# ericzzj1989/BALF

Measured on NVIDIA B200. Metric: images/sec detect+NMS+top-k @640x480, higher is better.
Workload: dtype fp16/tf32 operands (11-bit significand), fp32 accumulate

## Files before the change

### balf_b200/csrc/detector_tc.cuh

```cuda
#pragma once
#include <cuda_fp16.h>
#include "detector.cuh"
#include "umma.cuh"

namespace balf {
using namespace umma;

constexpr int kMerge32Ctas = 3;
constexpr int kRc16MinC = 32;
constexpr int TM = 128;
constexpr int NT2 = 256;
constexpr int kMaxSlot = 4;
constexpr int kMaxGemm = 6;

struct TcGemm {
    uint32_t goff;
    uint16_t nblk;
    uint16_t rows;
    uint16_t kb;
    uint16_t bias;
    uint16_t h16;
};
__host__ __device__ constexpr uint32_t tc_eb(int h16) { return h16 == 1 ? 2u : 4u; }
struct TcPlan {
    const float* base;
    TcGemm g[kMaxGemm];
    int ngemm;
    int resident;
    uint32_t bytes;
    uint32_t slot_bytes;
    uint32_t nslot;
    uint32_t ebias_off;
    long long* trace;
};
#ifdef BALF_TC_MAIN
long long* g_tc_trace = nullptr;
int g_tc_trace_sel = 0;
#else
extern long long* g_tc_trace;
extern int g_tc_trace_sel;
#endif
constexpr int kTracePoints = 16, kTraceTiles = 16;
#ifdef BALF_TC_TRACE
#define TC_TRACE(plan, it, pt)                                                                                     \
    do {                                                                                                           \
        if ((plan).trace && blockIdx.x == 0 && (it) < kTraceTiles && (threadIdx.x == 0 || threadIdx.x == NT2 - 1)) \
            (plan).trace[(((it) * kTracePoints + (pt)) << 1) + (threadIdx.x ? 1 : 0)] = clock64();                 \
    } while (0)
#else
#define TC_TRACE(plan, it, pt) do { (void)(it); } while (0)
#endif

enum { BG_CONV0 = 0, BG_PD1, BG_D1A, BG_D1B, BG_WM, BG_D2, BG_COUNT };
enum { MG_CONV0 = 0, MG_PD2A, MG_PD2B, MG_RC1, MG_RC2, MG_COUNT };
enum { HG_C2 = 0, HG_DENSE, HG_COUNT };
constexpr int kHeadN = 80;

__host__ __device__ constexpr int tc_kin(int cin) { return cin < 8 ? 8 : cin; }
__host__ __device__ constexpr int tc_kb(int rows, int K, int cap = 32768, int eb = 4) {
    int kb = K;
    while (kb > 32 / eb && (kb * rows * eb > cap || K % kb != 0)) kb /= 2;
    return kb;
}
__host__ __device__ constexpr int tc_cols(int need) { return need <= 32 ? 32 : need <= 64 ? 64 : need <= 128 ? 128 : need <= 256 ? 256 : 512; }
__host__ __device__ inline uint32_t gemm_block_bytes(const TcGemm& g, uint32_t b) {
    return (uint32_t)g.rows * (g.kb * tc_eb(g.h16) + ((g.bias && b + 1 == g.nblk) ? 32u : 0u));
}
__host__ __device__ inline uint32_t gemm_bytes(const TcGemm& g) {
    return (uint32_t)g.rows * ((uint32_t)g.kb * g.nblk * tc_eb(g.h16) + (g.bias ? 32u : 0u));
}

struct Ring {
    uint32_t wsm;
    uint64_t* full;
    uint64_t* empty;
    uint32_t pidx, nsched;
    const uint2* sched;
    uint32_t pcnt, ccnt;
    uint32_t pslot, puse;
    uint32_t cslot, cpar;
    uint32_t to_load;
};

__device__ __forceinline__ void bulk_load(uint32_t dst, const float* src, uint32_t bytes, uint64_t* bar) {
    asm volatile("cp.async.bulk.shared::cluster.global.mbarrier::complete_tx::bytes [%0], [%1], %2, [%3];"
                 :: "r"(dst), "l"(src), "r"(bytes), "r"(smem_u32(bar)) : "memory");
}
__device__ __forceinline__ void ring_build_schedule(uint2* sched, const TcPlan& p, uint32_t* count) {
    uint32_t n = 0;
    for (int gi = 0; gi < p.ngemm; ++gi) {
        const TcGemm g = p.g[gi];
        for (uint32_t b = 0; b < g.nblk; ++b)
            sched[n++] = make_uint2(g.goff + b * (uint32_t)g.rows * g.kb / (g.h16 == 1 ? 2u : 1u), gemm_block_bytes(g, b));
    }
    *count = n;
}
template <int NS>
__device__ __forceinline__ void ring_load_one(Ring& r, const TcPlan& p) {
    const uint2 e = r.sched[r.pidx];
    const uint32_t slot = r.pslot;
    if (r.puse > 0) mbar_wait(&r.empty[slot], (r.puse - 1) & 1);
    mbar_expect_tx(&r.full[slot], e.y);
    bulk_load(r.wsm + slot * p.slot_bytes, p.base + e.x, e.y, &r.full[slot]);
    ++r.pcnt;
    --r.to_load;
    if (++r.pslot == NS) { r.pslot = 0; ++r.puse; }
    if (++r.pidx == r.nsched) r.pidx = 0;
}
template <int NS>
__device__ __forceinline__ void ring_top_up(Ring& r, const TcPlan& p) {
    while (r.to_load > 0 && r.pcnt < r.ccnt + NS) ring_load_one<NS>(r, p);
}
template <int NS>
__device__ __forceinline__ void ring_consumed(Ring& r) {
    ++r.ccnt;
    if (++r.cslot == NS) { r.cslot = 0; r.cpar ^= 1; }
}
__device__ __forceinline__ void ring_load_all(Ring& r, const TcPlan& p) {
    mbar_expect_tx(&r.full[0], p.bytes);
    uint32_t off = 0;
    for (int gi = 0; gi < p.ngemm; ++gi) {
        const uint32_t bytes = gemm_bytes(p.g[gi]);
        bulk_load(r.wsm + off, p.base + p.g[gi].goff, bytes, &r.full[0]);
        off += bytes;
    }
}
template <int CIN, int C, int PX = 0> struct BranchG {
    static constexpr int count = BG_COUNT;
    static constexpr bool x3 = PX != 0;
    static constexpr bool resident = PX ? C <= 64 : C <= 128;
    static constexpr int cap = 32768;
    static constexpr int nslot = PX ? (C == 256 ? 2 : 3) : (C == 256 ? 3 : 2);
    __host__ __device__ static constexpr int rows(int gi) { return gi == BG_WM ? 64 : C; }
    __host__ __device__ static constexpr int K(int gi) { return gi == BG_CONV0 ? tc_kin(CIN) : gi == BG_WM ? 64 : C; }
    __host__ __device__ static constexpr bool bias(int gi) { return gi != BG_WM; }
    __host__ __device__ static constexpr bool h16(int gi) { return gi != BG_CONV0 || CIN >= 8; }
};
template <int CIN, int C, int PX = 0> struct MergeG {
    static constexpr int count = MG_COUNT;
    static constexpr bool x3 = PX != 0;
    static constexpr bool ebias = C == 128 && PX == 0;
    static constexpr bool resident = PX ? C <= 32 : C <= 128;
    static constexpr int cap = 32768;
    static constexpr int nslot = PX ? (C == 64 ? 3 : 2) : (C == 256 ? 2 : 3);
    __host__ __device__ static constexpr int rows(int) { return C; }
    __host__ __device__ static constexpr int K(int gi) { return gi == MG_CONV0 ? tc_kin(CIN) : C; }
    __host__ __device__ static constexpr bool bias(int gi) { return !ebias && gi != MG_PD2A; }
    __host__ __device__ static constexpr bool h16(int gi) {
        return gi == MG_PD2A || gi == MG_PD2B || (gi == MG_CONV0 && CIN >= 8) || ((gi == MG_RC1 || gi == MG_RC2) && (PX || C > kRc16MinC));
    }
};
template <int C, int PX = 0> struct HeadG {
    static constexpr int count = HG_COUNT;
    static constexpr bool x3 = PX != 0;
    static constexpr bool resident = false;
    static constexpr int cap = 32768;
    static constexpr int nslot = 2;
    __host__ __device__ static constexpr int rows(int gi) { return gi == HG_DENSE ? kHeadN : C; }
    __host__ __device__ static constexpr int K(int) { return C; }
    __host__ __device__ static constexpr bool bias(int) { return true; }
    __host__ __device__ static constexpr bool h16(int) { return true; }
};
template <typename G> __host__ __device__ constexpr int g_mode(int gi) { return G::h16(gi) ? (G::x3 ? 2 : 1) : 0; }
template <typename G> __host__ __device__ constexpr uint32_t g_bytes(int gi) {
    return (uint32_t)G::rows(gi) * (G::K(gi) * tc_eb(g_mode<G>(gi)) + (G::bias(gi) ? 32u : 0u));
}
template <typename G> __host__ __device__ constexpr uint32_t g_off(int gi) { uint32_t o = 0; for (int i = 0; i < gi; ++i) o += g_bytes<G>(i); return o; }

constexpr uint32_t kDescHi = (128u >> 4) | (1u << 14);
__device__ __forceinline__ uint64_t desc_of(uint32_t addr, uint32_t lbo) {
    return ((uint64_t)kDescHi << 32) | (uint64_t)(((lbo >> 4) << 16) | ((addr >> 4) & 0x3FFFu));
}

__host__ __device__ constexpr uint32_t make_idesc_f16(int M, int N) { return (1u << 4) | ((uint32_t)(N >> 3) << 17) | ((uint32_t)(M >> 4) << 24); }
__device__ __forceinline__ void mma_f16(uint32_t d_tmem, uint64_t a_desc, uint64_t b_desc, uint32_t idesc, bool accumulate) {
    asm volatile(
        "{\n\t.reg .pred p;\n\tsetp.ne.b32 p, %4, 0;\n\t"
        "tcgen05.mma.cta_group::1.kind::f16 [%0], %1, %2, %3, p;\n\t}"
        :: "r"(d_tmem), "l"(a_desc), "l"(b_desc), "r"(idesc), "r"((uint32_t)accumulate) : "memory");
}
constexpr uint32_t kDescHiSw = (1024u >> 4) | (1u << 14) | (2u << 29);
__device__ __forceinline__ uint64_t desc_sw_of(uint32_t addr) {
    return ((uint64_t)kDescHiSw << 32) | (uint64_t)((1u << 16) | ((addr >> 4) & 0x3FFFu));
}
template <typename G, int GI, bool ASW = false>
__device__ __forceinline__ void issue_linear_t(Ring& r, const TcPlan& p, uint32_t a_addr, uint32_t ones_addr, uint32_t d_tmem, bool first) {
    constexpr int ROWS = G::rows(GI), K = G::K(GI);
    constexpr bool BIAS = G::bias(GI), H16 = G::h16(GI);
    constexpr bool X3 = H16 && G::x3;
    static_assert(!(H16 && ASW), "fp16 operands use the chunk-major layout");
    constexpr int KB = tc_kb(ROWS, K, G::cap, (int)tc_eb(g_mode<G>(GI))), NBLK = K / KB;
    constexpr uint32_t idesc = H16 ? make_idesc_f16(128, ROWS) : make_idesc_tf32(128, ROWS);
    constexpr uint32_t a_lbo = TM * 16u, b_lbo = (uint32_t)ROWS * 16u;
    constexpr int KSTEP = H16 ? 16 : 8, EPC = H16 ? 8 : 4;
    const uint64_t a_desc = ASW ? desc_sw_of(a_addr) : desc_of(a_addr, a_lbo);
#pragma unroll
    for (int b = 0; b < NBLK; ++b) {
        uint32_t w_addr, slot = 0;
        if (G::resident) {
            w_addr = r.wsm + g_off<G>(GI) + (uint32_t)b * ROWS * KB * tc_eb(g_mode<G>(GI));
        } else {
            ring_top_up<G::nslot>(r, p);
            slot = r.cslot;
            mbar_wait(&r.full[slot], r.cpar);
            w_addr = r.wsm + slot * p.slot_bytes;
        }
        const uint64_t b_desc = desc_of(w_addr, b_lbo);
        fence_after_sync();
#pragma unroll
        for (int ks = 0; ks < KB / KSTEP; ++ks) {
            const uint32_t kchunk = (uint32_t)(b * KB) / EPC + (uint32_t)ks * 2u;
            const uint32_t a_off = ASW ? (kchunk / 8u) * (TM * 128u) + (kchunk % 8u) * 16u : kchunk * a_lbo;
            if (H16) mma_f16(d_tmem, a_desc + (a_off >> 4), b_desc + (((uint32_t)ks * 2u * b_lbo) >> 4), idesc, !(first && b == 0 && ks == 0));
            else mma_tf32(d_tmem, a_desc + (a_off >> 4), b_desc + (((uint32_t)ks * 2u * b_lbo) >> 4), idesc, !(first && b == 0 && ks == 0));
            if constexpr (X3) {
                mma_f16(d_tmem, a_desc + ((a_off + (uint32_t)(K / 8) * a_lbo) >> 4), b_desc + (((uint32_t)ks * 2u * b_lbo) >> 4), idesc, true);
                mma_f16(d_tmem, a_desc + (a_off >> 4), b_desc + ((((uint32_t)KB / 8u + (uint32_t)ks * 2u) * b_lbo) >> 4), idesc, true);
            }
        }
        if (BIAS && b + 1 == NBLK)
            mma_tf32(d_tmem, desc_of(ones_addr, TM * 16u), b_desc + ((((uint32_t)KB / EPC) * (X3 ? 2u : 1u) * b_lbo) >> 4), make_idesc_tf32(128, ROWS), true);
        if (!G::resident) { commit(&r.empty[slot]); ring_consumed<G::nslot>(r); }
    }
}

constexpr uint32_t kDescHiMn = ((uint32_t)(TM * 16u) >> 4) | (1u << 14);
__device__ __forceinline__ uint64_t desc_mn_of(uint32_t addr) {
    return ((uint64_t)kDescHiMn << 32) | (uint64_t)(((128u >> 4) << 16) | ((addr >> 4) & 0x3FFFu));
}
template <typename G, int GI, int C>
__device__ __forceinline__ void issue_mix_t(Ring& r, const TcPlan& p, uint32_t y_addr, uint32_t d_tmem) {
    uint32_t w_addr, slot = 0;
    if (G::resident) {
        w_addr = r.wsm + g_off<G>(GI);
    } else {
        ring_top_up<G::nslot>(r, p);
        slot = r.cslot;
        mbar_wait(&r.full[slot], r.cpar);
        w_addr = r.wsm + slot * p.slot_bytes;
    }
    fence_after_sync();
    constexpr uint32_t idesc = make_idesc_f16(64, C) | (1u << 16);
    constexpr uint32_t lo_off = (uint32_t)(C / 8) * TM * 16u;
    const uint64_t w_desc = desc_of(w_addr, 1024u);
    const uint64_t y_desc = desc_mn_of(y_addr);
#pragma unroll
    for (uint32_t u = 0; u < 2; ++u) {
#pragma unroll
        for (uint32_t ks = 0; ks < 4; ++ks) {
            const uint32_t yo = (32u * ks + 16u * u) * 16u;
            mma_f16(d_tmem + ((u * 16u) << 16), w_desc + ((ks * 2u * 1024u) >> 4), y_desc + (yo >> 4), idesc, ks > 0);
            if constexpr (G::x3) {
                mma_f16(d_tmem + ((u * 16u) << 16), w_desc + ((ks * 2u * 1024u) >> 4), y_desc + ((lo_off + yo) >> 4), idesc, true);
                mma_f16(d_tmem + ((u * 16u) << 16), w_desc + ((8192u + ks * 2u * 1024u) >> 4), y_desc + (yo >> 4), idesc, true);
            }
        }
    }
    if (!G::resident) { commit(&r.empty[slot]); ring_consumed<G::nslot>(r); }
}

__device__ __forceinline__ float ex2_approx(float x) {
    float y;
    asm("ex2.approx.ftz.f32 %0, %1;" : "=f"(y) : "f"(x));
    return y;
}
__device__ __forceinline__ unsigned long long pk2(float lo, float hi) {
    unsigned long long r;
    asm("mov.b64 %0, {%1, %2};" : "=l"(r) : "f"(lo), "f"(hi));
    return r;
}
__device__ __forceinline__ void upk2(unsigned long long r, float& lo, float& hi) { asm("mov.b64 {%0, %1}, %2;" : "=f"(lo), "=f"(hi) : "l"(r)); }
__device__ __forceinline__ unsigned long long fma2(unsigned long long a, unsigned long long b, unsigned long long c) {
    unsigned long long d;
    asm("fma.rn.f32x2 %0, %1, %2, %3;" : "=l"(d) : "l"(a), "l"(b), "l"(c));
    return d;
}
__device__ __forceinline__ unsigned long long add2(unsigned long long a, unsigned long long b) {
    unsigned long long d;
    asm("add.rn.f32x2 %0, %1, %2;" : "=l"(d) : "l"(a), "l"(b));
    return d;
}
__device__ __forceinline__ unsigned long long mul2(unsigned long long a, unsigned long long b) {
    unsigned long long d;
    asm("mul.rn.f32x2 %0, %1, %2;" : "=l"(d) : "l"(a), "l"(b));
    return d;
}
__device__ __forceinline__ void gelu_erf2(float& v0, float& v1) {
    const float t0 = fmaxf(-fabsf(v0), -5.6568542494923806f), t1 = fmaxf(-fabsf(v1), -5.6568542494923806f);
    const unsigned long long t = pk2(t0, t1);
    unsigned long long p = fma2(pk2(3.586947569e-04f, 3.586947569e-04f), t, pk2(6.316647399e-03f, 6.316647399e-03f));
    p = fma2(p, t, pk2(5.013782158e-02f, 5.013782158e-02f));
// ... 157 lines not shown
    uint64_t* bars = reinterpret_cast<uint64_t*>(q);
    s.full = bars;
    s.empty = bars + kMaxSlot;
    s.done = bars + 2 * kMaxSlot;
    s.aux = bars + 2 * kMaxSlot + 1;
    s.tmem_slot = reinterpret_cast<uint32_t*>(bars + 2 * kMaxSlot + 2);
    s.gdone = bars + 2 * kMaxSlot + 3;
    return s;
}

template <int NS>
__device__ __forceinline__ void tc_prologue(const TcShared& s, uint32_t ncols, Ring& ring, const TcPlan& plan, uint32_t my_tiles, bool w0) {
    if (threadIdx.x < 32) tmem_alloc(s.tmem_slot, ncols);
    if (threadIdx.x == 0) {
        for (int i = 0; i < kMaxSlot; ++i) { mbar_init(&s.full[i], 1); mbar_init(&s.empty[i], 1); }
        mbar_init(s.done, 1);
        mbar_init(s.aux, 1);
        for (int i = 0; i < kMaxGroups; ++i) mbar_init(&s.gdone[i], 1);
        mbar_fence_init();
    }
    for (int i = threadIdx.x; i < 2 * TM; i += blockDim.x)
        reinterpret_cast<float4*>(s.ones)[i] = i < TM ? make_float4(1.f, 1.f, 0.f, 0.f) : make_float4(0.f, 0.f, 0.f, 0.f);
    fence_async_smem();
    fence_before_sync();
    __syncthreads();
    fence_after_sync();
    ring.wsm = s.wsm; ring.full = s.full; ring.empty = s.empty; ring.sched = s.sched;
    ring.pidx = ring.pcnt = ring.ccnt = 0;
    ring.pslot = ring.puse = ring.cslot = ring.cpar = 0;
    uint32_t nb = 0;
    for (int i = 0; i < plan.ngemm; ++i) nb += plan.g[i].nblk;
    ring.nsched = nb;
    ring.to_load = nb * my_tiles;
    if (w0 && elect_one()) {
        if (plan.resident) { ring_load_all(ring, plan); mbar_wait(&s.full[0], 0); }
        else {
            uint32_t cnt;
            ring_build_schedule(s.sched, plan, &cnt);
            ring_top_up<NS>(ring, plan);
        }
    }
}
__device__ __forceinline__ void tc_finish(uint32_t tm, uint32_t ncols) {
    fence_before_sync();
    __syncthreads();
    if (threadIdx.x < 32) tmem_dealloc(tm, ncols);
}
template <int NG = 1, int NTG = NT2>
__device__ __forceinline__ void sync_for_mma(int grp = 0) {
    fence_async_smem();
    fence_before_sync();
    group_sync<NG, NTG>(grp);
    fence_after_sync();
}
__device__ __forceinline__ void wait_done(uint64_t* done, uint32_t& phase) {
    if (threadIdx.x == 0) mbar_wait(done, phase & 1);
    __syncthreads();
    ++phase;
    fence_after_sync();
}
template <typename G, int NG = 1, int NTG = NT2>
__device__ __forceinline__ void wait_done_ring(uint64_t* done, uint32_t& phase, Ring& r, const TcPlan& p, bool w0, int grp = 0) {
    if (w0 && elect_one()) {
        mbar_wait(done, phase & 1);
        if (!G::resident) ring_top_up<G::nslot>(r, p);
    }
// ... 326 lines not shown
    const uint32_t lane_base = tm + ((uint32_t)(row & ~31) << 16);
    const uint32_t region_addr = smem_u32(s.region), ones_addr = smem_u32(s.ones);
    const int ug = (row & 31) >> 4, tok = (row >> 5) * 16 + (row & 15);
    const int col0 = half * CH;
    const float* const mix_b1p = s.vec + 512 + tok;
    const int ostride = (BR == 0 ? geo.fw : 1) * C;
    const size_t npix = (size_t)geo.h * geo.w;
    uint32_t phase = 0, xb = 0;
    int it = 0;
    InputPf<CIN, TPR> pf;
    auto coords = [&](int tt, bool& vld, int& im, int& px) {
        const int un = 2 * tt + ug;
        vld = un < geo.total_units;
        im = vld ? fast_div(un, geo.upi, geo.inv_upi) : 0;
        px = unit_pixel<BR>(geo, vld ? un - im * geo.upi : 0, tok);
    };
    auto stats_of = [&](const float (&v)[CH], float& sum, float& sq) {
        unsigned long long s2 = pk2(0.f, 0.f), q2 = pk2(0.f, 0.f);
#pragma unroll
        for (int i = 0; i < CH; i += 2) {
            const unsigned long long x = pk2(v[i], v[i + 1]);
            s2 = add2(s2, x); q2 = fma2(x, x, q2);
        }
        float a, b;
        upk2(s2, a, b); sum = a + b;
        upk2(q2, a, b); sq = a + b;
    };
    bool nvld = false; int nim = 0, npx = 0;
    if (InputPf<CIN, TPR>::enabled && vblock < ntiles) {
        coords(vblock, nvld, nim, npx);
        fetch_input_row<CIN, true, TPR, XH>(xin, npix, (size_t)nim, npx, nvld, half, pf);
    }
    for (int t = vblock; t < ntiles; t += vgrid, ++it) {
        TC_TRACE(plan, it, 0);
        bool valid; int img, pix;
        if (InputPf<CIN, TPR>::enabled && (TPR > 1 || !X3)) { valid = nvld; img = nim; pix = npx; }
        else coords(t, valid, img, pix);
        float* orow = rt + ((size_t)img * npix + pix) * C + col0;
        float v[CH], rstd, shift;
        if constexpr (CIN < 8) {
            const float4 xv = pf.v[0];
            if (t + vgrid < ntiles) {
                coords(t + vgrid, nvld, nim, npx);
                fetch_input_row<CIN, true, TPR, XH>(xin, npix, (size_t)nim, npx, nvld, half, pf);
            }
            conv0_row<CIN, C, CH>(xv, s.vec, col0, v);
        } else {
            if (InputPf<CIN, TPR>::enabled) {
                store_input_row<CIN, true, TPR, XM>(pf, s.region, row, half);
                if (t + vgrid < ntiles) {
                    coords(t + vgrid, nvld, nim, npx);
                    fetch_input_row<CIN, true, TPR, XH>(xin, npix, (size_t)nim, npx, nvld, half, pf);
                }
            } else {
                load_input_row<CIN, TPR, XM>(xin, npix, (size_t)img, pix, valid, s.region, row, half);
            }
            TC_TRACE(plan, it, 1);
            sync_for_mma<NG, NTG>(grp);
            if (w0 && elect_one()) { issue_linear_t<G, BG_CONV0>(ring, plan, region_addr, ones_addr, tm + Cfg::col_y, true); commit(s.done); }
            TC_TRACE(plan, it, 2);
            wait_done_ring<G, NG, NTG>(s.done, phase, ring, plan, w0, grp);
            TC_TRACE(plan, it, 3);
            ld_row<CH>(lane_base + Cfg::col_y + col0, v);
#pragma unroll
            for (int i = 0; i < CH; ++i) v[i] = fmaxf(v[i], 0.f);
        }
// ... 140 lines not shown
                        float4 t8[8];
                        pair_load<8>(reinterpret_cast<const float4*>(orow + c) + j0, valid, t8);
#pragma unroll
                        for (int j = 0; j < 8; j += 2) { pair_unswap(t8[j], t8[j + 1]); rq[j0 + j] = t8[j]; rq[j0 + j + 1] = t8[j + 1]; }
                    }
                }
#pragma unroll
                for (int j = 0; j < SC / 4; ++j) {
                    float4 res;
                    res = make_float4(r[4 * j], r[4 * j + 1], r[4 * j + 2], r[4 * j + 3]);
                    o[j] = make_float4(a[4 * j] + res.x, a[4 * j + 1] + res.y, a[4 * j + 2] + res.z, a[4 * j + 3] + res.w);
                    if (BR == 1 && !X3) o[j] = to_tf32_clean(o[j]);
                }
                if constexpr (SC % 32 == 0 && !X3) {
                    oct_store<SC / 4>(out, ((size_t)img * npix + pix) * C + col0 + c, ostride, reinterpret_cast<const float*>(o), valid);
                    continue;
                }
#pragma unroll
                for (int j = 0; j < SC / 4; j += 2) {
                    const float4 send = odd ? o[j] : o[j + 1];
                    float4 recv;
                    recv.x = __shfl_xor_sync(0xffffffffu, send.x, 1); recv.y = __shfl_xor_sync(0xffffffffu, send.y, 1);
                    recv.z = __shfl_xor_sync(0xffffffffu, send.z, 1); recv.w = __shfl_xor_sync(0xffffffffu, send.w, 1);
                    const float4 to_a = odd ? recv : o[j], to_b = odd ? o[j + 1] : recv;
                    const int chunk = (col0 + c) / 4 + j + (odd ? 1 : 0);
                    if (valid) {
                        *reinterpret_cast<float4*>(out + base_a + 4 * chunk) = to_a;
                        *reinterpret_cast<float4*>(out + base_b + 4 * chunk) = to_b;
                    }
                }
            }
        }
    }
    tc_finish(*s.tmem_slot, tc_cols(Cfg::ncols * NG));
}

template <int CIN, int C, int BR, int PX>
__global__ void __launch_bounds__(BranchCfg<C, PX>::NTG * BranchCfg<C, PX>::groups, 1)
tc_branch_kernel(const float* __restrict__ xin, DownW w, TcPlan plan, UnitGeom geo, float* __restrict__ out, float* __restrict__ scratch) {
    extern __shared__ __align__(1024) unsigned char smem[];
    tc_branch_body<CIN, C, BR, PX>(xin, w, plan, geo, out, scratch, smem);
}


template <int C, int NTH = NT2>
__device__ __forceinline__ void unit_channel_sums(const float* reg, int t, int total_units, float* __restrict__ partial) {
    constexpr int CQ = C / 4, PAIRS = 2 * CQ, TPP = NTH / PAIRS, RPT = 64 / TPP;
    static_assert(TPP >= 2 && TPP <= 16, "group must fit in a warp");
    const int tid = threadIdx.x, pair = tid / TPP, sub = tid % TPP;
    const int uu = pair / CQ, ch = pair % CQ;
    const float4* src = reinterpret_cast<const float4*>(reg) + (size_t)ch * TM + uu * 64 + sub;
    float4 acc = src[0];
#pragma unroll
    for (int i = 1; i < RPT; ++i) {
        const float4 x = src[i * TPP];
        acc.x += x.x; acc.y += x.y; acc.z += x.z; acc.w += x.w;
    }
#pragma unroll
    for (int o = TPP / 2; o >= 1; o >>= 1) {
        acc.x += __shfl_xor_sync(0xffffffffu, acc.x, o);
        acc.y += __shfl_xor_sync(0xffffffffu, acc.y, o);
        acc.z += __shfl_xor_sync(0xffffffffu, acc.z, o);
        acc.w += __shfl_xor_sync(0xffffffffu, acc.w, o);
    }
    const int un = 2 * t + uu;
    if (sub == 0 && un < total_units) *reinterpret_cast<float4*>(partial + (size_t)un * C + ch * 4) = acc;
// ... 42 lines not shown
    }
    const float* const eb = s.vec + col0_of(tid, CH);
    const uint32_t lane_base = tm + ((uint32_t)(row & ~31) << 16);
    const uint32_t region_addr = smem_u32(s.region), ones_addr = smem_u32(s.ones);
    const uint32_t r2_addr = region_addr + Cfg::r2_off;
    uint64_t* const ld_u = s.aux;
    uint64_t* const ld_v = &s.gdone[1];
    constexpr uint32_t kTileBytes = Cfg::uv_bytes;
    const size_t tile_floats = (size_t)kTileBytes / 4;
    uint32_t ld_phase = 0;
    const int ug = row >> 6, tok = row & 63;
    const int col0 = half * CH;
    const size_t npix = (size_t)geo.h * geo.w;
    uint32_t phase = 0, xb = 0;
    int it = 0;
    InputPf<CIN, TPR> pf;
    InputPf<C> pfu;
    auto coords = [&](int tt, bool& vld, int& im, int& px) {
        const int un = 2 * tt + ug;
        vld = un < geo.total_units;
        im = vld ? fast_div(un, geo.upi, geo.inv_upi) : 0;
        px = (vld ? un - im * geo.upi : 0) * 64 + tok;
    };
    if (InputPf<CIN, TPR>::enabled && (int)blockIdx.x < ntiles) {
        bool vld; int im, px;
        coords(blockIdx.x, vld, im, px);
        fetch_input_row<CIN, true, TPR, XH>(xin, npix, (size_t)im, px, vld, half, pf);
    }
    if (Cfg::bulk_uv && (int)blockIdx.x < ntiles && w0 && elect_one()) {
        mbar_expect_tx(ld_u, kTileBytes);
        bulk_load(r2_addr, uin + (size_t)blockIdx.x * tile_floats, kTileBytes, ld_u);
    }
    for (int t = blockIdx.x; t < ntiles; t += gridDim.x, ++it) {
        TC_TRACE(plan, it, 0);
        bool valid; int img, pix;
        coords(t, valid, img, pix);
        const size_t row_off = ((size_t)img * npix + pix) * C + col0;
        float v[CH];
        if (InputPf<CIN, TPR>::enabled) {
            store_input_row<CIN, true, TPR, XM>(pf, s.region, row, half);
            if (t + (int)gridDim.x < ntiles) {
                bool vld; int im, px;
                coords(t + gridDim.x, vld, im, px);
                fetch_input_row<CIN, true, TPR, XH>(xin, npix, (size_t)im, px, vld, half, pf);
            }
        } else {
            load_input_row<CIN, TPR, XM>(xin, npix, (size_t)img, pix, valid, s.region, row, half, PX ? 0 : CIN);
        }
        if (InputPf<C>::enabled) fetch_input_row<C>(uin, npix, (size_t)img, pix, valid, half, pfu);
        TC_TRACE(plan, it, 1);
        sync_for_mma();
        if constexpr (Cfg::bulk_uv) {
            if (w0 && elect_one()) {
                issue_linear_t<G, MG_CONV0>(ring, plan, region_addr, ones_addr, tm + Cfg::col_x0, true);
                mbar_wait(ld_u, ld_phase & 1);
                fence_after_sync();
                issue_linear_t<G, MG_PD2A>(ring, plan, r2_addr, ones_addr, tm + Cfg::col_acc, true);
                commit(s.done);
            }
            wait_done_ring<G>(s.done, phase, ring, plan, w0);
            if (w0 && elect_one()) {
                mbar_expect_tx(ld_v, kTileBytes);
                bulk_load(region_addr, vin + (size_t)t * tile_floats, kTileBytes, ld_v);
                if (!Cfg::two && t + (int)gridDim.x < ntiles) {
                    mbar_expect_tx(ld_u, kTileBytes);
                    bulk_load(r2_addr, uin + (size_t)(t + gridDim.x) * tile_floats, kTileBytes, ld_u);
// ... 99 lines not shown
            const float4 o = make_float4(v[4 * j], v[4 * j + 1], v[4 * j + 2], v[4 * j + 3]);
            *reinterpret_cast<float4*>(s.region + ((size_t)(col0 / 4 + j) * TM + row) * 4) = o;
        }
        static_assert(PX != 0 || C < 128 || CH % 64 == 0, "the fp16 r store (r16, decided by the host) assumes two threads per row");
        if constexpr (CH % 64 == 0 && PX == 0) {
            if (r16) {
                float hv[CH / 2];
#pragma unroll
                for (int i = 0; i < CH / 2; ++i) {
                    uint32_t h;
                    asm("cvt.rn.satfinite.f16x2.f32 %0, %1, %2;" : "=r"(h) : "f"(v[2 * i + 1]), "f"(v[2 * i]));
                    hv[i] = __uint_as_float(h);
                }
                oct_store<CH / 8>(rout, row_off / 2, C / 2, hv, valid);
            } else {
                oct_store<CH / 4>(rout, row_off, C, v, valid);
            }
        } else if constexpr (CH % 32 == 0 && PX == 0) {
            oct_store<CH / 4>(rout, row_off, C, v, valid);
        } else {
            pair_store<CH / 4>(rout, row_off, v, valid);
        }
        __syncthreads();
        unit_channel_sums<C, NTK>(s.region, t, geo.total_units, partial);
        if constexpr (Cfg::two) fence_async_smem();
        __syncthreads();
        if constexpr (Cfg::two) {
            if (t + (int)gridDim.x < ntiles && w0 && elect_one()) {
                mbar_expect_tx(ld_u, kTileBytes);
                bulk_load(r2_addr, uin + (size_t)(t + gridDim.x) * tile_floats, kTileBytes, ld_u);
            }
        }
    }
    tc_finish(tm, Cfg::ncols);
}


template <int CIN, int C, int PX = 0> struct MergeBulkCfg {
    static constexpr int CH = C / 2;
    static constexpr bool cc0 = CIN < 8;
    static constexpr uint32_t tile_bytes = (uint32_t)TM * C * 4;
    static constexpr uint32_t uv_bytes = (uint32_t)TM * C * (PX ? 4u : 2u);
    static constexpr uint32_t r16_bytes = 0u;
    static constexpr uint32_t xbytes = cc0 ? 0u : (uint32_t)TM * tc_kin(CIN) * 4;
    static constexpr uint32_t region = 2 * uv_bytes + r16_bytes + 2 * tile_bytes + xbytes;
    static constexpr uint32_t xch = 2u * TM * 8u;
    static constexpr int col_acc = 0, col_x0 = C;
    static constexpr int ncols = tc_cols(cc0 ? C : 2 * C);
    static constexpr int min_ctas = C <= 32 ? (PX ? 2 : kMerge32Ctas) : 1;
};

template <int CIN, int C, int PX = 0>
__global__ void __launch_bounds__(NT2, MergeBulkCfg<CIN, C, PX>::min_ctas)
tc_merge_bulk_kernel(const float* __restrict__ xin, DownW w, TcPlan plan, UnitGeom geo, const float* __restrict__ uin,
                     const float* __restrict__ vin, float* __restrict__ rout, float* __restrict__ qout, float* __restrict__ partial) {
    extern __shared__ __align__(1024) unsigned char smem[];
    using Cfg = MergeBulkCfg<CIN, C, PX>;
    constexpr int CH = Cfg::CH;
    using G = MergeG<CIN, C, PX>;
    constexpr int HM = PX ? 2 : 1, LOC = PX ? C / 8 : 0;
    constexpr bool XH = PX == 0 && CIN >= 8;
    constexpr int XM = XH ? 3 : HM;
    const TcShared s = carve(smem, Cfg::region, plan, 1, Cfg::xch);
    float* const regU = s.region;
    float* const regV = regU + Cfg::uv_bytes / 4;
    float* const regW = regV + Cfg::uv_bytes / 4;
// ... 152 lines not shown
            bulk_commit();
        }
        {
            constexpr int CQ = C / 4, TPP = NT2 / (2 * CQ), RPT = 64 / TPP;
            const int pair = tid / TPP, sub = tid % TPP;
            const int uu = pair / CQ, ch = pair % CQ;
            float4 acc = *reinterpret_cast<const float4*>(regW + sw_off(uu * 64 + sub, ch));
#pragma unroll
            for (int i = 1; i < RPT; ++i) {
                const float4 x = *reinterpret_cast<const float4*>(regW + sw_off(uu * 64 + sub + i * TPP, ch));
                acc.x += x.x; acc.y += x.y; acc.z += x.z; acc.w += x.w;
            }
#pragma unroll
            for (int o = TPP / 2; o >= 1; o >>= 1) {
                acc.x += __shfl_xor_sync(0xffffffffu, acc.x, o);
                acc.y += __shfl_xor_sync(0xffffffffu, acc.y, o);
                acc.z += __shfl_xor_sync(0xffffffffu, acc.z, o);
                acc.w += __shfl_xor_sync(0xffffffffu, acc.w, o);
            }
            if (sub == 0) *reinterpret_cast<float4*>(partial + (size_t)(2 * t + uu) * C + ch * 4) = acc;
        }
    }
    if (w0 && elect_one()) bulk_wait_all();
    tc_finish(tm, Cfg::ncols);
}

template <int C, int PX = 0>
__global__ void __launch_bounds__(NT2, 1) tc_head_kernel(const float* __restrict__ r, const float* __restrict__ q,
                                                         const float* __restrict__ scale, TcPlan plan, UnitGeom geo, int cell,
                                                         float* __restrict__ logits, float* __restrict__ prob, int r16) {
    extern __shared__ __align__(1024) unsigned char smem[];
    using G = HeadG<C, PX>;
    constexpr int LOC = PX ? C / 8 : 0;
    constexpr uint32_t region_bytes = (uint32_t)TM * C * 4;
    constexpr int ncols = tc_cols(C + 96);
    constexpr int CH = C / 2;
    const TcShared s = carve(smem, region_bytes, plan);
    const int tid = threadIdx.x, row = tid & (TM - 1), half = tid >> 7;
    const int ntiles = (geo.total_units + 1) / 2;
    const uint32_t my_tiles = blockIdx.x < (unsigned)ntiles ? (ntiles - 1 - blockIdx.x) / gridDim.x + 1 : 0;
    Ring ring;
    const bool w0 = warp0_uniform();
    tc_prologue<G::nslot>(s, ncols, ring, plan, my_tiles, w0);
    const uint32_t tm = *s.tmem_slot;
    const uint32_t lane_base = tm + ((uint32_t)(row & ~31) << 16);
    const uint32_t region_addr = smem_u32(s.region), ones_addr = smem_u32(s.ones);
    const int ug = row >> 6, tok = row & 63;
    const int col0 = half * CH;
    const size_t npix = (size_t)geo.h * geo.w;
    const int nlog = cell * cell + 1;
    uint32_t phase = 0;
    for (int t = blockIdx.x; t < ntiles; t += gridDim.x) {
        const int unit = 2 * t + ug;
        const bool valid = unit < geo.total_units;
        const int img = valid ? fast_div(unit, geo.upi, geo.inv_upi) : 0, u = valid ? unit - img * geo.upi : 0;
        const int pix = u * 64 + tok;
        const size_t row_off = ((size_t)img * npix + pix) * C + col0;
#pragma unroll 1
        for (int j0 = 0; j0 < CH / 4; j0 += 8) {
            float4 rv[8], qv[8];
            if constexpr (PX == 0) {
                if (r16) {
                    const uint4* rh = reinterpret_cast<const uint4*>(reinterpret_cast<const __half*>(r) + row_off) + j0 / 2;
#pragma unroll
                    for (int k = 0; k < 4; ++k) {
                        const uint4 h = valid ? __ldg(rh + k) : make_uint4(0u, 0u, 0u, 0u);
                        const float2 a = __half22float2(*reinterpret_cast<const __half2*>(&h.x)), b = __half22float2(*reinterpret_cast<const __half2*>(&h.y));
                        const float2 c2 = __half22float2(*reinterpret_cast<const __half2*>(&h.z)), d = __half22float2(*reinterpret_cast<const __half2*>(&h.w));
                        rv[2 * k] = make_float4(a.x, a.y, b.x, b.y);
                        rv[2 * k + 1] = make_float4(c2.x, c2.y, d.x, d.y);
                    }
                } else {
                    oct_load<8>(r, row_off + (size_t)j0 * 4, C, valid, rv);
                }
                oct_load<8>(q, row_off + (size_t)j0 * 4, C, valid, qv);
            } else {
                pair_load<8>(reinterpret_cast<const float4*>(r + row_off) + j0, valid, rv);
                pair_load<8>(reinterpret_cast<const float4*>(q + row_off) + j0, valid, qv);
#pragma unroll
                for (int j = 0; j < 8; j += 2) { pair_unswap(rv[j], rv[j + 1]); pair_unswap(qv[j], qv[j + 1]); }
            }
#pragma unroll
            for (int j = 0; j < 8; j += 2) {
                float e[8];
#pragma unroll
                for (int u2 = 0; u2 < 2; ++u2) {
                    const float4 sv = __ldg(reinterpret_cast<const float4*>(scale + (size_t)img * C + col0) + j0 + j + u2);
                    e[4 * u2] = rv[j + u2].x * sv.x + qv[j + u2].x; e[4 * u2 + 1] = rv[j + u2].y * sv.y + qv[j + u2].y;
                    e[4 * u2 + 2] = rv[j + u2].z * sv.z + qv[j + u2].z; e[4 * u2 + 3] = rv[j + u2].w * sv.w + qv[j + u2].w;
                }
                uint32_t h[4], l[4];
#pragma unroll
                for (int w2 = 0; w2 < 4; ++w2) {
                    if constexpr (PX) split_h2(e[2 * w2], e[2 * w2 + 1], h[w2], l[w2]);
                    else asm("cvt.rn.satfinite.f16x2.f32 %0, %1, %2;" : "=r"(h[w2]) : "f"(e[2 * w2 + 1]), "f"(e[2 * w2]));
                }
                *reinterpret_cast<uint4*>(s.region + ((size_t)((col0 / 4 + j0 + j) / 2) * TM + row) * 4) = make_uint4(h[0], h[1], h[2], h[3]);
                if constexpr (PX)
                    *reinterpret_cast<uint4*>(s.region + ((size_t)(LOC + (col0 / 4 + j0 + j) / 2) * TM + row) * 4) = make_uint4(l[0], l[1], l[2], l[3]);
            }
        }
        sync_for_mma();
        if (w0 && elect_one()) { issue_linear_t<G, HG_C2>(ring, plan, region_addr, ones_addr, tm, true); commit(s.done); }
        wait_done_ring<G>(s.done, phase, ring, plan, w0);
        {
            float v[CH];
            ld_row<CH>(lane_base + col0, v);
#pragma unroll
            for (int i = 0; i < CH; ++i) v[i] = fmaxf(v[i], 0.f);
            row_to_a16<CH, LOC>(v, s.region, row, col0);
        }
        sync_for_mma();
        if (w0 && elect_one()) { issue_linear_t<G, HG_DENSE>(ring, plan, region_addr, ones_addr, tm + C, true); commit(s.done); }
        wait_done_ring<G>(s.done, phase, ring, plan, w0);
        if (half == 0) {
            float z[96];
            ld_row<96>(lane_base + C, z);
            float mx = kNegInf;
#pragma unroll
            for (int n = 0; n < 65; ++n) mx = fmaxf(mx, z[n]);
            float den = 0.f;
#pragma unroll
            for (int n = 0; n < 65; ++n) den += expf(z[n] - mx);
            if (valid) {
                const int cy = pix / geo.w, cx = pix - cy * geo.w;
                const int Wp = geo.w * cell, Hp = geo.h * cell;
                if (logits) {
#pragma unroll
                    for (int n = 0; n < 65; ++n) logits[((size_t)img * nlog + n) * npix + pix] = z[n];
                }
                const float inv = 1.0f / den;
                if (cell == 8) {
#pragma unroll
                    for (int n = 0; n < 64; n += 4) {
                        const int yy = cy * 8 + (n >> 3), xx = cx * 8 + (n & 7);
                        *reinterpret_cast<float4*>(prob + ((size_t)img * Hp + yy) * Wp + xx) =
                            make_float4(expf(z[n] - mx) * inv, expf(z[n + 1] - mx) * inv, expf(z[n + 2] - mx) * inv, expf(z[n + 3] - mx) * inv);
                    }
                } else {
#pragma unroll
                for (int n = 0; n < 64; ++n) {
                    const int yy = cy * cell + (n >> 3), xx = cx * cell + (n & 7);
                    prob[((size_t)img * Hp + yy) * Wp + xx] = expf(z[n] - mx) * inv;
                }
                }
            }
        }
    }
    tc_finish(tm, ncols);
}

#ifdef BALF_TC_MAIN
__global__ void tc_pack_kernel(const float* __restrict__ wT, int ld, int n0, int rows, int k_real, int k_pad, int kb,
                               const float* __restrict__ gamma, const float* __restrict__ alpha, float* __restrict__ dst) {
    const int i = blockIdx.x * blockDim.x + threadIdx.x;
    if (i >= rows * k_pad) return;
    const int k = i / rows, n = i - k * rows;
    const int b = k / kb, kk = k - b * kb;
    float v = 0.f;
    if (k < k_real) {
        v = wT[(size_t)k * ld + n0 + n];
        if (gamma) v *= gamma[k];
        if (alpha) v *= alpha[n0 + n];
    }
    dst[(size_t)b * rows * kb + (size_t)(kk >> 2) * rows * 4 + n * 4 + (kk & 3)] = to_tf32_exact(v);
}
__global__ void tc_pack_h16_kernel(const float* __restrict__ wT, int ld, int n0, int rows, int k_real, int k_pad, int kb,
                                   const float* __restrict__ gamma, const float* __restrict__ alpha, __half* __restrict__ dst) {
    const int i = blockIdx.x * blockDim.x + threadIdx.x;
    if (i >= rows * k_pad) return;
    const int k = i / rows, n = i - k * rows;
    const int b = k / kb, kk = k - b * kb;
    float v = 0.f;
    if (k < k_real) {
        v = wT[(size_t)k * ld + n0 + n];
        if (gamma) v *= gamma[k];
        if (alpha) v *= alpha[n0 + n];
    }
    dst[(size_t)b * rows * kb + (size_t)(kk >> 3) * rows * 8 + n * 8 + (kk & 7)] = __float2half_rn(v);
}
__global__ void tc_pack_x3_kernel(const float* __restrict__ wT, int ld, int n0, int rows, int k_real, int k_pad, int kb,
// ... 77 lines not shown
    TcPlans P;
    const int hm = px ? 2 : 1;
    for (int l = 0; l < 4; ++l) {
        const int cin = tc_kin(a.dims[l]), c = a.dims[l + 1];
        for (int b = 0; b < 2; ++b) {
            TcPlan& p = P.branch[l][b];
            p = TcPlan{};
            p.base = base; p.ngemm = BG_COUNT;
            p.resident = px ? c <= 64 : c <= 128;
            p.nslot = px ? (c == 256 ? 2 : 3) : (c == 256 ? 3 : 2);
            tc_add(p, BG_CONV0, off, c, cin, true, 32768, a.dims[l] >= 8 ? hm : 0);
            tc_add(p, BG_PD1, off, c, c, true, 32768, hm);
            tc_add(p, BG_D1A, off, c, c, true, 32768, hm);
            tc_add(p, BG_D1B, off, c, c, true, 32768, hm);
            tc_add(p, BG_WM, off, 64, 64, false, 32768, hm);
            tc_add(p, BG_D2, off, c, c, true, 32768, hm);
        }
        TcPlan& m = P.merge[l];
        m = TcPlan{};
        m.base = base; m.ngemm = MG_COUNT;
        m.resident = px ? c <= 32 : c <= 128;
        m.nslot = px ? (c == 64 ? 3 : 2) : (c == 256 ? 2 : 3);
        const int mcap = 32768;
        const bool ebias = c == 128 && !px;
        tc_add(m, MG_CONV0, off, c, cin, !ebias, mcap, a.dims[l] >= 8 ? hm : 0);
        tc_add(m, MG_PD2A, off, c, c, false, mcap, hm);
        tc_add(m, MG_PD2B, off, c, c, !ebias, mcap, hm);
        tc_add(m, MG_RC1, off, c, c, !ebias, mcap, (px || c > kRc16MinC) ? hm : 0);
        tc_add(m, MG_RC2, off, c, c, !ebias, mcap, (px || c > kRc16MinC) ? hm : 0);
        if (ebias) { m.ebias_off = (uint32_t)off; off += (size_t)4 * c * 4; }
    }
    TcPlan& h = P.head;
    h = TcPlan{};
    h.base = base; h.ngemm = HG_COUNT; h.resident = 0; h.nslot = 2;
    tc_add(h, HG_C2, off, a.dims[4], a.dims[4], true, 32768, hm);
    tc_add(h, HG_DENSE, off, kHeadN, a.dims[4], true, 32768, hm);
    P.floats = off;
    for (int l = 0; l < 4; ++l) {
        P.branch[l][0].trace = P.branch[l][1].trace = g_tc_trace_sel == 0 ? g_tc_trace : nullptr;
        P.merge[l].trace = g_tc_trace_sel == 1 ? g_tc_trace : nullptr;
    }
    P.head.trace = nullptr;
    if (out) *out = P;
}
static void tc_build_plans(const balf_detector_arch& a, const float* base, TcPlans* out, int px = 0) {
    size_t off = 0;
    TcPlans P0;
    tc_build_plans_px(a, base, &P0, 0, off);
    if (px) tc_build_plans_px(a, base, out, 1, off);
    else if (out) *out = P0;
}

#ifdef BALF_TC_MAIN
size_t tc_blob_floats(const balf_detector_arch& a) {
    TcPlans P;
    tc_build_plans(a, nullptr, &P, 1);
    return P.floats;
}

struct Fold { const float* gamma; const float* beta; const float* alpha; const float* add; };

static void tc_pack_one(const TcPlan& p, int gi, const float* wT, int ld, int n0, int k_real, const float* bias, Fold f,
                        float* blob, cudaStream_t st) {
    const TcGemm& g = p.g[gi];
    const int k_pad = g.nblk * g.kb;
    if (g.h16 == 2)
        tc_pack_x3_kernel<<<cdiv(g.rows * k_pad, 256), 256, 0, st>>>(wT, ld, n0, g.rows, k_real, k_pad, g.kb, f.gamma, f.alpha,
                                                                     reinterpret_cast<__half*>(blob + g.goff));
    else if (g.h16)
        tc_pack_h16_kernel<<<cdiv(g.rows * k_pad, 256), 256, 0, st>>>(wT, ld, n0, g.rows, k_real, k_pad, g.kb, f.gamma, f.alpha,
                                                                      reinterpret_cast<__half*>(blob + g.goff));
    else
        tc_pack_kernel<<<cdiv(g.rows * k_pad, 256), 256, 0, st>>>(wT, ld, n0, g.rows, k_real, k_pad, g.kb, f.gamma, f.alpha, blob + g.goff);
    if (g.bias)
        tc_pack_bias_kernel<<<cdiv(g.rows, 128), 128, 0, st>>>(wT, ld, n0, g.rows, k_real, bias, f.beta, f.alpha, f.add,
// ... 112 lines not shown
    } else {
        const TcPlan& p = P.merge[level];
        BALF_REQUIRE((!MergeCfg<C, PX>::bulk_uv || g.total_units % 2 == 0), "internal: odd unit count at stage %d", level);
        const size_t smem = tc_smem_bytes(MergeCfg<C, PX>::region, p, 1, MergeCfg<C, PX>::xch);
        if (int e = tc_launch_cfg(tc_merge_kernel<CIN, C, PX>, smem, MergeCfg<C, PX>::ncols, ntiles, &grid, 1, MergeCfg<C, PX>::NT)) return e;
        ProfScope ps(C == 128 ? "det_merge_c128" : "det_merge_c256", st);
        tc_merge_kernel<CIN, C, PX><<<grid, MergeCfg<C, PX>::NT, smem, st>>>(xin, p, g, u, v, r, q, partial, r16);
    }
    BALF_COUNT_LAUNCH(3);
    BALF_LAUNCH_OK();
    return 0;
}

template <int PX>
int tc_level_px(int level, const float* xin, const DownW& w, const balf_detector_arch& a, const float* blob,
                int Bc, int h, int wd, float* u, float* v, float* r, float* q, float* partial, cudaStream_t st, int r16) {
    TcPlans P;
    tc_build_plans(a, blob, &P, PX);
    switch (level) {
        case 0: return tc_run_level<3, 32, PX>(xin, w, P, 0, Bc, h, wd, u, v, r, q, partial, st, r16);
        case 1: return tc_run_level<32, 64, PX>(xin, w, P, 1, Bc, h, wd, u, v, r, q, partial, st, r16);
        case 2: return tc_run_level<64, 128, PX>(xin, w, P, 2, Bc, h, wd, u, v, r, q, partial, st, r16);
        default: return tc_run_level<128, 256, PX>(xin, w, P, 3, Bc, h, wd, u, v, r, q, partial, st, r16);
    }
}
template <int PX>
int tc_head_px(const float* r, const float* q, const float* scale, const balf_detector_arch& a,
               const float* blob, int Bc, int hc, int wc, float* logits, float* prob, cudaStream_t st, int r16) {
    TcPlans P;
    tc_build_plans(a, blob, &P, PX);
    UnitGeom g{hc, wc, hc / 8, wc / 8, hc * wc / 64, Bc * (hc * wc / 64), 1.0f / (float)(hc * wc / 64), 1.0f / (float)(wc / 8), 1.0f / (float)(wc / 8)};
    BALF_REQUIRE(g.total_units < (1 << 23), "internal: %d units in one pass exceed the fast_div range", g.total_units);
    const int ntiles = (g.total_units + 1) / 2;
    const size_t smem = tc_smem_bytes((uint32_t)TM * 256 * 4, P.head);
    int grid = 0;
    BALF_REQUIRE((plan_matches<HeadG<256, PX>>(P.head)), "internal: compile-time and packed GEMM plans differ (head)");
    if (int e = tc_launch_cfg(tc_head_kernel<256, PX>, smem, 512, ntiles, &grid)) return e;
    {
        ProfScope ps("det_head", st);
        tc_head_kernel<256, PX><<<grid, NT2, smem, st>>>(r, q, scale, P.head, g, a.cell, logits, prob, PX ? 0 : r16);
    }
    BALF_COUNT_LAUNCH(1);
    BALF_LAUNCH_OK();
    return 0;
}

#ifdef BALF_TC_MAIN
extern template int tc_level_px<1>(int, const float*, const DownW&, const balf_detector_arch&, const float*, int, int, int, float*, float*,
                                   float*, float*, float*, cudaStream_t, int);
extern template int tc_head_px<1>(const float*, const float*, const float*, const balf_detector_arch&, const float*, int, int, int, float*,
                                  float*, cudaStream_t, int);

int tc_run_level_dispatch(int level, const float* xin, const DownW& w, const balf_detector_arch& a, const float* blob,
                          int Bc, int h, int wd, float* u, float* v, float* r, float* q, float* partial, cudaStream_t st, int px, int r16) {
    return px ? tc_level_px<1>(level, xin, w, a, blob, Bc, h, wd, u, v, r, q, partial, st, r16)
              : tc_level_px<0>(level, xin, w, a, blob, Bc, h, wd, u, v, r, q, partial, st, r16);
}

int tc_run_head(const float* r, const float* q, const float* scale, const balf_detector_arch& a,
                const float* blob, int Bc, int hc, int wc, float* logits, float* prob, cudaStream_t st, int px, int r16) {
    return px ? tc_head_px<1>(r, q, scale, a, blob, Bc, hc, wc, logits, prob, st, r16)
              : tc_head_px<0>(r, q, scale, a, blob, Bc, hc, wc, logits, prob, st, r16);
}
#endif

}

// ... 7 lines not shown
```

Before: 5241.

## Deepen head weight ring, refill slots behind consumption, shrink fp16 head region

For the non-x3 head kernel, the weight ring grows from two to three slots. The A region is sized for fp16 (2 bytes per element) instead of 4, which frees the shared memory the extra slot needs. Rings with three or more slots now refill right after a slot is consumed rather than topping up before each wait, so weight loads run further ahead of the MMAs. Trace-only instrumentation of mbarrier wait cycles and head-kernel trace points is also added; it compiles out by default. The risks are a shared-memory change that could alter occupancy, and the refill change also affecting merge and branch rings that already use three slots.

```diff
diff --git a/balf_b200/csrc/detector_tc.cuh b/balf_b200/csrc/detector_tc.cuh
--- a/balf_b200/csrc/detector_tc.cuh
+++ b/balf_b200/csrc/detector_tc.cuh
@@ -41,14 +41,27 @@
 extern int g_tc_trace_sel;
 #endif
 constexpr int kTracePoints = 16, kTraceTiles = 16;
+constexpr int kTraceWaitOff = 2 * kTracePoints * kTraceTiles;
 #ifdef BALF_TC_TRACE
 #define TC_TRACE(plan, it, pt)                                                                                     \
     do {                                                                                                           \
         if ((plan).trace && blockIdx.x == 0 && (it) < kTraceTiles && (threadIdx.x == 0 || threadIdx.x == NT2 - 1)) \
             (plan).trace[(((it) * kTracePoints + (pt)) << 1) + (threadIdx.x ? 1 : 0)] = clock64();                 \
     } while (0)
+#define TC_TRACE_WAITS(plan, r, it)                                                                                \
+    do {                                                                                                           \
+        if ((plan).trace && blockIdx.x == 0 && (it) >= 0 && (it) < kTraceTiles && (r).ccnt > 0) {                 \
+            (plan).trace[kTraceWaitOff + 2 * (it)] = (r).wait_full;                                                \
+            (plan).trace[kTraceWaitOff + 2 * (it) + 1] = (r).wait_empty;                                           \
+        }                                                                                                          \
+        (r).wait_full = (r).wait_empty = 0;                                                                        \
+    } while (0)
+#define TC_TIMED_WAIT(bar, par, acc)                                                                               \
+    do { const long long t0_ = clock64(); mbar_wait(bar, par); (acc) += clock64() - t0_; } while (0)
 #else
 #define TC_TRACE(plan, it, pt) do { (void)(it); } while (0)
+#define TC_TRACE_WAITS(plan, r, it) do { (void)(it); } while (0)
+#define TC_TIMED_WAIT(bar, par, acc) mbar_wait(bar, par)
 #endif
 
 enum { BG_CONV0 = 0, BG_PD1, BG_D1A, BG_D1B, BG_WM, BG_D2, BG_COUNT };
@@ -80,6 +93,9 @@
     uint32_t pslot, puse;
     uint32_t cslot, cpar;
     uint32_t to_load;
+#ifdef BALF_TC_TRACE
+    long long wait_full, wait_empty;
+#endif
 };
 
 __device__ __forceinline__ void bulk_load(uint32_t dst, const float* src, uint32_t bytes, uint64_t* bar) {
@@ -99,7 +115,7 @@
 __device__ __forceinline__ void ring_load_one(Ring& r, const TcPlan& p) {
     const uint2 e = r.sched[r.pidx];
     const uint32_t slot = r.pslot;
-    if (r.puse > 0) mbar_wait(&r.empty[slot], (r.puse - 1) & 1);
+    if (r.puse > 0) TC_TIMED_WAIT(&r.empty[slot], (r.puse - 1) & 1, r.wait_empty);
     mbar_expect_tx(&r.full[slot], e.y);
     bulk_load(r.wsm + slot * p.slot_bytes, p.base + e.x, e.y, &r.full[slot]);
     ++r.pcnt;
@@ -110,6 +126,11 @@
 template <int NS>
 __device__ __forceinline__ void ring_top_up(Ring& r, const TcPlan& p) {
     while (r.to_load > 0 && r.pcnt < r.ccnt + NS) ring_load_one<NS>(r, p);
+}
+template <int NS> constexpr bool kRefillBehind = NS >= 3;
+template <int NS>
+__device__ __forceinline__ void ring_refill_behind(Ring& r, const TcPlan& p) {
+    while (r.to_load > 0 && r.pcnt + 1 < r.ccnt + NS) ring_load_one<NS>(r, p);
 }
 template <int NS>
 __device__ __forceinline__ void ring_consumed(Ring& r) {
@@ -155,7 +176,7 @@
     static constexpr bool x3 = PX != 0;
     static constexpr bool resident = false;
     static constexpr int cap = 32768;
-    static constexpr int nslot = 2;
+    static constexpr int nslot = PX ? 2 : 3;
     __host__ __device__ static constexpr int rows(int gi) { return gi == HG_DENSE ? kHeadN : C; }
     __host__ __device__ static constexpr int K(int) { return C; }
     __host__ __device__ static constexpr bool bias(int) { return true; }
@@ -200,9 +221,9 @@
         if (G::resident) {
             w_addr = r.wsm + g_off<G>(GI) + (uint32_t)b * ROWS * KB * tc_eb(g_mode<G>(GI));
         } else {
-            ring_top_up<G::nslot>(r, p);
+            if constexpr (!kRefillBehind<G::nslot>) ring_top_up<G::nslot>(r, p);
             slot = r.cslot;
-            mbar_wait(&r.full[slot], r.cpar);
+            TC_TIMED_WAIT(&r.full[slot], r.cpar, r.wait_full);
             w_addr = r.wsm + slot * p.slot_bytes;
         }
         const uint64_t b_desc = desc_of(w_addr, b_lbo);
@@ -220,7 +241,11 @@
         }
         if (BIAS && b + 1 == NBLK)
             mma_tf32(d_tmem, desc_of(ones_addr, TM * 16u), b_desc + ((((uint32_t)KB / EPC) * (X3 ? 2u : 1u) * b_lbo) >> 4), make_idesc_tf32(128, ROWS), true);
-        if (!G::resident) { commit(&r.empty[slot]); ring_consumed<G::nslot>(r); }
+        if (!G::resident) {
+            commit(&r.empty[slot]);
+            ring_consumed<G::nslot>(r);
+            if constexpr (kRefillBehind<G::nslot>) ring_refill_behind<G::nslot>(r, p);
+        }
     }
 }
 
@@ -234,9 +259,9 @@
     if (G::resident) {
         w_addr = r.wsm + g_off<G>(GI);
     } else {
-        ring_top_up<G::nslot>(r, p);
+        if constexpr (!kRefillBehind<G::nslot>) ring_top_up<G::nslot>(r, p);
         slot = r.cslot;
-        mbar_wait(&r.full[slot], r.cpar);
+        TC_TIMED_WAIT(&r.full[slot], r.cpar, r.wait_full);
         w_addr = r.wsm + slot * p.slot_bytes;
     }
     fence_after_sync();
@@ -256,7 +281,11 @@
             }
         }
     }
-    if (!G::resident) { commit(&r.empty[slot]); ring_consumed<G::nslot>(r); }
+    if (!G::resident) {
+        commit(&r.empty[slot]);
+        ring_consumed<G::nslot>(r);
+        if constexpr (kRefillBehind<G::nslot>) ring_refill_behind<G::nslot>(r, p);
+    }
 }
 
 __device__ __forceinline__ float ex2_approx(float x) {
@@ -480,6 +509,9 @@
     for (int i = 0; i < plan.ngemm; ++i) nb += plan.g[i].nblk;
     ring.nsched = nb;
     ring.to_load = nb * my_tiles;
+#ifdef BALF_TC_TRACE
+    ring.wait_full = ring.wait_empty = 0;
+#endif
     if (w0 && elect_one()) {
         if (plan.resident) { ring_load_all(ring, plan); mbar_wait(&s.full[0], 0); }
         else {
@@ -872,6 +904,7 @@
         fetch_input_row<CIN, true, TPR, XH>(xin, npix, (size_t)nim, npx, nvld, half, pf);
     }
     for (int t = vblock; t < ntiles; t += vgrid, ++it) {
+        TC_TRACE_WAITS(plan, ring, it - 1);
         TC_TRACE(plan, it, 0);
         bool valid; int img, pix;
         if (InputPf<CIN, TPR>::enabled && (TPR > 1 || !X3)) { valid = nvld; img = nim; pix = npx; }
@@ -1078,6 +1111,7 @@
             }
         }
     }
+    TC_TRACE_WAITS(plan, ring, it - 1);
     tc_finish(*s.tmem_slot, tc_cols(Cfg::ncols * NG));
 }
 
@@ -1186,6 +1220,7 @@
         bulk_load(r2_addr, uin + (size_t)blockIdx.x * tile_floats, kTileBytes, ld_u);
     }
     for (int t = blockIdx.x; t < ntiles; t += gridDim.x, ++it) {
+        TC_TRACE_WAITS(plan, ring, it - 1);
         TC_TRACE(plan, it, 0);
         bool valid; int img, pix;
         coords(t, valid, img, pix);
@@ -1351,6 +1386,7 @@
             }
         }
     }
+    TC_TRACE_WAITS(plan, ring, it - 1);
     tc_finish(tm, Cfg::ncols);
 }
 
@@ -1569,7 +1605,7 @@
     extern __shared__ __align__(1024) unsigned char smem[];
     using G = HeadG<C, PX>;
     constexpr int LOC = PX ? C / 8 : 0;
-    constexpr uint32_t region_bytes = (uint32_t)TM * C * 4;
+    constexpr uint32_t region_bytes = (uint32_t)TM * C * (PX ? 4 : 2);
     constexpr int ncols = tc_cols(C + 96);
     constexpr int CH = C / 2;
     const TcShared s = carve(smem, region_bytes, plan);
@@ -1587,7 +1623,10 @@
     const size_t npix = (size_t)geo.h * geo.w;
     const int nlog = cell * cell + 1;
     uint32_t phase = 0;
-    for (int t = blockIdx.x; t < ntiles; t += gridDim.x) {
+    int it = 0;
+    for (int t = blockIdx.x; t < ntiles; t += gridDim.x, ++it) {
+        TC_TRACE_WAITS(plan, ring, it - 1);
+        TC_TRACE(plan, it, 0);
         const int unit = 2 * t + ug;
         const bool valid = unit < geo.total_units;
         const int img = valid ? fast_div(unit, geo.upi, geo.inv_upi) : 0, u = valid ? unit - img * geo.upi : 0;
@@ -1637,9 +1676,12 @@
                     *reinterpret_cast<uint4*>(s.region + ((size_t)(LOC + (col0 / 4 + j0 + j) / 2) * TM + row) * 4) = make_uint4(l[0], l[1], l[2], l[3]);
             }
         }
+        TC_TRACE(plan, it, 1);
         sync_for_mma();
         if (w0 && elect_one()) { issue_linear_t<G, HG_C2>(ring, plan, region_addr, ones_addr, tm, true); commit(s.done); }
+        TC_TRACE(plan, it, 2);
         wait_done_ring<G>(s.done, phase, ring, plan, w0);
+        TC_TRACE(plan, it, 3);
         {
             float v[CH];
             ld_row<CH>(lane_base + col0, v);
@@ -1647,9 +1689,12 @@
             for (int i = 0; i < CH; ++i) v[i] = fmaxf(v[i], 0.f);
             row_to_a16<CH, LOC>(v, s.region, row, col0);
         }
+        TC_TRACE(plan, it, 4);
         sync_for_mma();
         if (w0 && elect_one()) { issue_linear_t<G, HG_DENSE>(ring, plan, region_addr, ones_addr, tm + C, true); commit(s.done); }
+        TC_TRACE(plan, it, 5);
         wait_done_ring<G>(s.done, phase, ring, plan, w0);
+        TC_TRACE(plan, it, 6);
         if (half == 0) {
             float z[96];
             ld_row<96>(lane_base + C, z);
@@ -1684,6 +1729,7 @@
             }
         }
     }
+    TC_TRACE_WAITS(plan, ring, it - 1);
     tc_finish(tm, ncols);
 }
 
@@ -1827,7 +1873,7 @@
     }
     TcPlan& h = P.head;
     h = TcPlan{};
-    h.base = base; h.ngemm = HG_COUNT; h.resident = 0; h.nslot = 2;
+    h.base = base; h.ngemm = HG_COUNT; h.resident = 0; h.nslot = px ? 2 : 3;
     tc_add(h, HG_C2, off, a.dims[4], a.dims[4], true, 32768, hm);
     tc_add(h, HG_DENSE, off, kHeadN, a.dims[4], true, 32768, hm);
     P.floats = off;
@@ -1835,7 +1881,7 @@
         P.branch[l][0].trace = P.branch[l][1].trace = g_tc_trace_sel == 0 ? g_tc_trace : nullptr;
         P.merge[l].trace = g_tc_trace_sel == 1 ? g_tc_trace : nullptr;
     }
-    P.head.trace = nullptr;
+    P.head.trace = g_tc_trace_sel == 2 ? g_tc_trace : nullptr;
     if (out) *out = P;
 }
 static void tc_build_plans(const balf_detector_arch& a, const float* base, TcPlans* out, int px = 0) {
@@ -2014,7 +2060,7 @@
     UnitGeom g{hc, wc, hc / 8, wc / 8, hc * wc / 64, Bc * (hc * wc / 64), 1.0f / (float)(hc * wc / 64), 1.0f / (float)(wc / 8), 1.0f / (float)(wc / 8)};
     BALF_REQUIRE(g.total_units < (1 << 23), "internal: %d units in one pass exceed the fast_div range", g.total_units);
     const int ntiles = (g.total_units + 1) / 2;
-    const size_t smem = tc_smem_bytes((uint32_t)TM * 256 * 4, P.head);
+    const size_t smem = tc_smem_bytes((uint32_t)TM * 256 * (PX ? 4 : 2), P.head);
     int grid = 0;
     BALF_REQUIRE((plan_matches<HeadG<256, PX>>(P.head)), "internal: compile-time and packed GEMM plans differ (head)");
     if (int e = tc_launch_cfg(tc_head_kernel<256, PX>, smem, 512, ntiles, &grid)) return e;
```

Result: faster. 5294, median of 6 (+1.0%).
